# ChristianFeldmann/VTM

Hardware: AMD Instinct MI355X
Metric: hot-path pictures/sec (3840x2160 randomaccess QP32; level-order predInterSearch: AMVP estimation, TZ + fractional ME per (list, refIdx), bi refinement, MC, residual xT/quant/xIT/SSE; not a full encode) + SATD Gblocks/s (higher is better)
Workload: dtype int16 samples, int32 accumulation (fp64 MV-rate multiply)

## Files before the change

### include/vtmhip.h

```cpp
#ifndef VTMHIP_H
#define VTMHIP_H

#include <stddef.h>
#include <stdint.h>

#ifdef __cplusplus
extern "C" {
#endif

#define VTMHIP_ABI_VERSION 6

enum
{
  VTMHIP_OK            = 0,
  VTMHIP_E_INVALID     = -1,
  VTMHIP_E_NODEVICE    = -2,
  VTMHIP_E_HIP         = -3,
  VTMHIP_E_NOMEM       = -4,
  VTMHIP_E_UNSUPPORTED = -5
};

enum { VTMHIP_DIST_SAD = 0, VTMHIP_DIST_SATD = 1, VTMHIP_DIST_SSE = 2 };
enum { VTMHIP_DCT2 = 0, VTMHIP_DCT8 = 1, VTMHIP_DST7 = 2,
       VTMHIP_TRSKIP = 3 };
// ... 694 lines not shown

typedef struct
{
  const int16_t *org;
  const int16_t *dpb;
  int16_t *pred, *resi;
  int16_t *orgBi;
  int16_t *predC, *resiC;
} vtmhip_pis_buffers;

int vtmhip_pis_run_picture( vtmhip_ctx *ctx, const vtmhip_pis_level_run *levels, int numLevels, const vtmhip_pis_buffers *buf, void *mainStream,
                            void *const *sideStreams, int numSide );

int vtmhip_predInterSearch_batch_dev( vtmhip_ctx *ctx, const vtmhip_pis_level_run *L, const vtmhip_pis_buffers *buf );
int vtmhip_is_uniform_shape( int width, int height );

#ifdef __cplusplus
}
#endif
#endif
```

### vtm_amd/csrc/me.hip

```cpp
#include "ctx.hpp"
#include "mest_glue.hpp"
#include "mv_rules.hpp"

#include <cstdlib>

namespace
{

struct Range { int left, right, top, bottom; };

struct MeJob
{
  const int16_t *org;
  const int16_t *ref;
  int            orgStride, refStride, w, h, ss;
  unsigned       imvShift;
  int            predHor, predVer, costScale;
  double         lambda;
  int            horMin, horMax, verMin, verMax;
  int            seg, segsPerRow, items, lpc;
  int            lpcShift, sprShift;
  bool           narrow;
  bool           tiny;
  unsigned       bias;
// ... 222 lines not shown

struct TzState
{
  Range              sr;
  unsigned long long bestSad;
  int                bestX, bestY, pointNr;
  unsigned           bestDist, bestRound, nEval;
};

struct Coop
{
  int                 lane, wave, wpj;
  bool                leader;
  unsigned long long *redCost;
  unsigned           *redIdx;
};

template<int WPJ>
__device__ __forceinline__ void job_sync()
{
  if( WPJ == 1 )
  {
    __builtin_amdgcn_fence( __ATOMIC_ACQ_REL, "wavefront" );
    __builtin_amdgcn_wave_barrier();
  }
  else
  {
    __syncthreads();
  }
}
// ... 115 lines not shown
    if( lane == 0 ) { co.redCost[co.wave] = bestCost; co.redIdx[co.wave] = bestIdx; }
    __syncthreads();
#pragma unroll
    for( int w = 0; w < WPJ; w++ )
    {
      const unsigned long long oc = co.redCost[w];
      const unsigned           oi = co.redIdx[w];
      if( oc < bestCost || ( oc == bestCost && oi < bestIdx ) ) { bestCost = oc; bestIdx = oi; }
    }
    __syncthreads();
  }
  bestCost = uni( bestCost );
  bestIdx  = uni( bestIdx );
}

template<int WPJ>
__device__ __forceinline__ void tz_round( const MeJob &j, TzState &s, const int4 *pts, int n, const Coop &co, bool touchMeta )
{
  job_sync<WPJ>();
  unsigned long long cost;
  unsigned           idx;
  eval_candidates<false, WPJ>( j, pts, n, 0, 0, 1, 1, co, cost, idx );
  s.nEval += ( unsigned ) n;
  if( n > 0 && cost < s.bestSad )
  {
    const int4 p = pts[idx];
    s.bestSad    = cost;
    s.bestX      = uni( p.x );
    s.bestY      = uni( p.y );
    if( touchMeta )
    {
      s.bestDist  = ( unsigned ) uni( p.w );
      s.bestRound = 0;
      s.pointNr   = uni( p.z );
    }
  }
  job_sync<WPJ>();
}

#define PUSH( X, Y, NR, D ) do { if( co.leader ) pts[n] = make_int4( ( X ), ( Y ), ( NR ), ( D ) ); n++; } while( 0 )

__device__ int diamond_points( const Range &sr, int sx, int sy, int d, bool corners, int4 *pts, const Coop &co )
{
  int       n = 0;
  const int top = sy - d, bot = sy + d, left = sx - d, right = sx + d;
  if( d == 1 )
  {
    if( top >= sr.top )
    {
      if( corners && left >= sr.left ) PUSH( left, top, 1, d );
      PUSH( sx, top, 2, d );
      if( corners && right <= sr.right ) PUSH( right, top, 3, d );
// ... 53 lines not shown
      if( inside || yt >= sr.top )
      {
        if( inside || xl >= sr.left ) PUSH( xl, yt, 0, d );
        if( inside || xr <= sr.right ) PUSH( xr, yt, 0, d );
      }
      if( inside || yb <= sr.bottom )
      {
        if( inside || xl >= sr.left ) PUSH( xl, yb, 0, d );
        if( inside || xr <= sr.right ) PUSH( xr, yb, 0, d );
      }
    }
  }
  return n;
}

template<int WPJ>
__device__ __forceinline__ void tz_diamond( const MeJob &j, TzState &s, int sx, int sy, int d, bool corners, int4 *pts, const Coop &co )
{
  const int n = diamond_points( s.sr, sx, sy, d, corners, pts, co );
  s.bestRound += 1;
  tz_round<WPJ>( j, s, pts, n, co, true );
}

template<int WPJ>
__device__ __forceinline__ void tz_two_point( const MeJob &j, TzState &s, int4 *pts, const Coop &co )
{
  const int xo0[9] = { 0, -1, -1, 0, -1, +1, -1, -1, +1 }, xo1[9] = { 0, 0, +1, +1, -1, +1, 0, +1, 0 };
  const int yo0[9] = { 0, 0, -1, -1, +1, -1, 0, +1, 0 }, yo1[9] = { 0, -1, -1, 0, -1, +1, +1, +1, +1 };
  int       ax = 0, ay = 0, bx = 0, by = 0;
#pragma unroll
  for( int k = 0; k < 9; k++ )
    if( k == s.pointNr ) { ax = xo0[k]; ay = yo0[k]; bx = xo1[k]; by = yo1[k]; }
  const int x1 = s.bestX + ax, y1 = s.bestY + ay, x2 = s.bestX + bx, y2 = s.bestY + by;
  int       n  = 0;
  if( x1 >= s.sr.left && x1 <= s.sr.right && y1 >= s.sr.top && y1 <= s.sr.bottom ) PUSH( x1, y1, 0, 2 );
  if( x2 >= s.sr.left && x2 <= s.sr.right && y2 >= s.sr.top && y2 <= s.sr.bottom ) PUSH( x2, y2, 0, 2 );
  tz_round<WPJ>( j, s, pts, n, co, true );
}

template<int IPL, int WPJ>
__device__ __forceinline__ void raster_resident_org( const MeJob &j, int total, int rLeft, int rTop, int nx, int stepXY, const Coop &co,
                                                     unsigned long long &bestCost, unsigned &bestIdx )
{
  const int lane = co.lane;
  const long os = ( long ) j.orgStride << j.ss, cs = ( long ) j.refStride << j.ss;
  Pel8 o[IPL];
  int  off[IPL];
#pragma unroll
  for( int m = 0; m < IPL; m++ )
  {
    const int it = lane + 64 * m, r = it >> j.sprShift, x = ( it - ( r << j.sprShift ) ) << 3;
    o[m] = *reinterpret_cast<const Pel8 *>( j.org + r * os + x );
// ... 28 lines not shown
    if( lane == 0 ) { co.redCost[co.wave] = bestCost; co.redIdx[co.wave] = bestIdx; }
    __syncthreads();
#pragma unroll
    for( int w = 0; w < WPJ; w++ )
    {
      const unsigned long long oc = co.redCost[w];
      const unsigned           oi = co.redIdx[w];
      if( oc < bestCost || ( oc == bestCost && oi < bestIdx ) ) { bestCost = oc; bestIdx = oi; }
    }
    __syncthreads();
  }
  bestCost = uni( bestCost );
  bestIdx  = uni( bestIdx );
}

template<int WPJ>
__device__ __forceinline__ void tz_raster( const MeJob &j, TzState &s, const Range &r, int stepXY, const Coop &co )
{
  const int nx = r.right >= r.left ? ( r.right - r.left ) / stepXY + 1 : 0;
  const int ny = r.bottom >= r.top ? ( r.bottom - r.top ) / stepXY + 1 : 0;
  const int total = nx * ny;
  unsigned long long cost;
  unsigned           idx;
  const int  ipl  = j.items >> 6;
  const bool fits = total > 0 && j.lpc == 64 && j.seg == 8 && j.sprShift >= 0 && ( j.items & 63 ) == 0;
  if( false ) {}
  else if( WPJ >= 4 && fits && ipl == 4 ) raster_resident_org<4, WPJ>( j, total, r.left, r.top, nx, stepXY, co, cost, idx );
  else if( WPJ >= 2 && fits && ipl == 1 ) raster_resident_org<1, WPJ>( j, total, r.left, r.top, nx, stepXY, co, cost, idx );
  else eval_candidates<true, WPJ>( j, nullptr, total, r.left, r.top, nx > 0 ? nx : 1, stepXY, co, cost, idx );
  s.nEval += ( unsigned ) total;
  if( total > 0 && cost < s.bestSad )
  {
    const int ry = ( int ) idx / nx, rx = ( int ) idx - ry * nx;
    s.bestSad   = cost;
    s.bestX     = r.left + rx * stepXY;
    s.bestY     = r.top + ry * stepXY;
    s.bestDist  = ( unsigned ) stepXY;
    s.bestRound = 0;
    s.pointNr   = 0;
  }
}

struct TzSaved
// ... 197 lines not shown
      if( c < bc ) { bc = c; bi = ( unsigned ) i; }
    }
    wave_argmin( bc, bi );
    if( lane == 0 ) { sRedCost[wv] = bc; sRedIdx[wv] = bi; }
    __syncthreads();
    if( threadIdx.x == 0 )
    {
      for( int w = 1; w < 4; w++ )
        if( sRedCost[w] < bc || ( sRedCost[w] == bc && sRedIdx[w] < bi ) ) { bc = sRedCost[w]; bi = sRedIdx[w]; }
      sv.rasterCost = bc; sv.rasterIdx = bi;
    }
    __syncthreads();
  }
}

template<int WPJ>
__device__ __forceinline__ void tz_search_one( const vtmhip_pic_params &pic, const int16_t *__restrict__ orgBase, const int16_t *__restrict__ refBase,
                                               const vtmhip_tz_job *__restrict__ jobs, int numJobs, vtmhip_me_result *__restrict__ results, int mode, TzSaved *__restrict__ saved,
                                               int *__restrict__ list, int totCap, const MeFuse &fu, int blockIdxX, int gridDimX )
{
  constexpr int JOBS_PER_BLOCK = WPJ == 1 ? 4 : 1;
  __shared__ int4               sPts[JOBS_PER_BLOCK][16];
  __shared__ unsigned long long sRedCost[WPJ];
  __shared__ unsigned           sRedIdx[WPJ];
  __shared__ __attribute__( ( aligned( 16 ) ) ) int16_t sOrgLds[WPJ >= 4 ? ORG_LDS_CAP : WPJ == 2 ? ORG_LDS_CAP2 : 8];
  const int lane = threadIdx.x & 63, wv = uni( ( int ) ( threadIdx.x >> 6 ) );
  const int blk    = mode == 2 ? blockIdxX : xcd_order( blockIdxX, gridDimX );
  int       jobIdx = WPJ == 1 ? blk * 4 + wv : blk;
  if( mode == 2 )
  {
    if( jobIdx >= list[0] ) return;
    jobIdx = uni( list[1 + jobIdx] );
  }
  if( jobIdx >= numJobs ) return;
  __shared__ int sExtra[JOBS_PER_BLOCK][15][2];
  vtmhip_tz_job  tj;
  const int( *extra )[2];
// ... 43 lines not shown
    const vtmhip_tz_job *jp = jobs + jobIdx;
    if( uni( ( int ) jp->width ) == 0 ) return;
    tj.orgOff = jp->orgOff; tj.refOff = jp->refOff; tj.orgStride = jp->orgStride; tj.refStride = jp->refStride; tj.puX = jp->puX; tj.puY = jp->puY;
    tj.width = jp->width; tj.height = jp->height; tj.subShift = jp->subShift; tj.imvShift = jp->imvShift; tj.signedSamples = jp->signedSamples;
    tj.predHor = jp->predHor; tj.predVer = jp->predVer; tj.motionLambda = jp->motionLambda; tj.mvHor = jp->mvHor; tj.mvVer = jp->mvVer; tj.searchRange = jp->searchRange;
    tj.extendedSettings = jp->extendedSettings; tj.fastSettings = jp->fastSettings; tj.firstSearchStop = jp->firstSearchStop; tj.hasIntMv2Nx2NPred = jp->hasIntMv2Nx2NPred;
    tj.intMv2Nx2NPredHor = jp->intMv2Nx2NPredHor; tj.intMv2Nx2NPredVer = jp->intMv2Nx2NPredVer;
    numExtra = jp->numExtraStart;
    extra = jp->extraStart;
  }
  const vtmhip_tz_job *jp = &tj;
  int4                *pts = sPts[WPJ == 1 ? wv : 0];
  Coop                 co;
  co.lane = lane; co.wave = WPJ == 1 ? 0 : wv; co.wpj = WPJ; co.leader = ( lane == 0 && co.wave == 0 );
  co.redCost = sRedCost; co.redIdx = sRedIdx;

  MeJob j;
  j.org       = orgBase + jp->orgOff;
  j.ref       = refBase + jp->refOff;
  j.orgStride = jp->orgStride;
  j.refStride = jp->refStride;
  j.w         = jp->width;
  j.h         = jp->height;
  j.ss        = jp->subShift;
  j.imvShift  = ( unsigned ) jp->imvShift;
  j.predHor   = jp->predHor;
  j.predVer   = jp->predVer;
  j.costScale = 2;
  j.lambda    = jp->motionLambda;
  j.horMax    = MVR_CLIP_MAX( pic.picW, jp->puX );
// ... 20 lines not shown
    const int  r = j.sprShift >= 0 ? sub >> j.sprShift : sub / j.segsPerRow, x = ( sub - r * j.segsPerRow ) * j.seg;
    const long os = ( long ) j.orgStride << j.ss;
    if( j.seg == 8 )
    {
      const Pel8 a = *reinterpret_cast<const Pel8 *>( j.org + r * os + x );
#pragma unroll
      for( int k = 0; k < 4; k++ ) j.orgSeg[k] = a.v[k] ^ j.bias;
    }
    else
    {
      const Pel4 a = *reinterpret_cast<const Pel4 *>( j.org + r * os + x );
      j.orgSeg[0] = a.v[0] ^ j.bias; j.orgSeg[1] = a.v[1] ^ j.bias;
    }
    j.resOff = ( int ) ( r * ( ( long ) j.refStride << j.ss ) + x );
  }
  stage_org<WPJ, ( WPJ >= 4 ? ORG_LDS_CAP : ORG_LDS_CAP2 )>( j, sOrgLds, ( int ) threadIdx.x );

  const bool ext = jp->extendedSettings != 0, fast = jp->fastSettings != 0, firstStop = jp->firstSearchStop != 0;
  const int  iRaster = fast ? 8 : 5, searchRange = jp->searchRange;

  TzState s;
  s.bestSad = ~0ull; s.bestX = 0; s.bestY = 0; s.pointNr = 0; s.bestDist = 0; s.bestRound = 0; s.nEval = 0;
  s.sr.left = s.sr.right = s.sr.top = s.sr.bottom = 0;

  int startX = 0, startY = 0;
  if( mode != 2 )
  {
  int mx = jp->mvHor, my = jp->mvVer;
  clip_mv( j, mx, my );
  mx = div_pow2( mvr::prec_down( mx, 2 ), 2 );
  my = div_pow2( mvr::prec_down( my, 2 ), 2 );
  if( !jp->hasIntMv2Nx2NPred )
  {
    int n = 0;
    PUSH( mx, my, 0, 0 );
    if( !fast && ( mx != 0 || my != 0 ) ) PUSH( 0, 0, 0, 0 );
    const int ne = min( numExtra, 14 );
    for( int i = 0; i < ne; i++ )
    {
      int ex = extra[i][0], ey = extra[i][1];
      clip_mv( j, ex, ey );
      PUSH( mvr::prec_down( ex, 4 ), mvr::prec_down( ey, 4 ), 0, 0 );
    }
    tz_round<WPJ>( j, s, pts, n, co, true );
    if( numExtra > 14 )
    {
      int m = 0;
      {
        int n = 0;
        int ex = extra[14][0], ey = extra[14][1];
        clip_mv( j, ex, ey );
        PUSH( mvr::prec_down( ex, 4 ), mvr::prec_down( ey, 4 ), 0, 0 );
        m = n;
      }
      tz_round<WPJ>( j, s, pts, m, co, false );
    }
  }
  else
  {
    {
      int n = 0;
      PUSH( mx, my, 0, 0 );
      tz_round<WPJ>( j, s, pts, n, co, true );
    }
    if( !fast && ( mx != 0 || my != 0 ) && ( s.bestX != 0 || s.bestY != 0 ) )
    {
      int n = 0;
      PUSH( 0, 0, 0, 0 );
      tz_round<WPJ>( j, s, pts, n, co, true );
    }
    int ix = jp->intMv2Nx2NPredHor << 4, iy = jp->intMv2Nx2NPredVer << 4;
    clip_mv( j, ix, iy );
    ix = div_pow2( mvr::prec_down( ix, 2 ), 2 );
    iy = div_pow2( mvr::prec_down( iy, 2 ), 2 );
    if( ( mx != ix || my != iy ) && ( ix != s.bestX || iy != s.bestY ) )
    {
      int n = 0;
      PUSH( ix, iy, 0, 0 );
      tz_round<WPJ>( j, s, pts, n, co, true );
    }
    int       n  = 0;
    const int ne = min( numExtra, 15 );
    for( int i = 0; i < ne; i++ )
    {
      int ex = extra[i][0], ey = extra[i][1];
      clip_mv( j, ex, ey );
      PUSH( mvr::prec_down( ex, 4 ), mvr::prec_down( ey, 4 ), 0, 0 );
    }
    tz_round<WPJ>( j, s, pts, n, co, false );
  }

  s.sr = search_range( j, s.bestX << 4, s.bestY << 4, searchRange >> ( fast ? 1 : 0 ) );

  startX = s.bestX; startY = s.bestY;
  const bool bestCandidateZero = ( s.bestX == 0 && s.bestY == 0 );

  for( int d = 1; d <= searchRange; d *= 2 )
  {
    tz_diamond<WPJ>( j, s, startX, startY, d, ext, pts, co );
    if( firstStop && s.bestRound >= 3 ) break;
  }
  if( ext && !bestCandidateZero )
  {
    for( int d = 1; d <= ( searchRange >> 1 ); d *= 2 ) tz_diamond<WPJ>( j, s, 0, 0, d, false, pts, co );
  }
  if( s.bestDist == 1 )
  {
    s.bestDist = 0;
    tz_two_point<WPJ>( j, s, pts, co );
  }
  if( ext )
  {
    int   win = iRaster;
    Range lsr = s.sr;
    if( !( ( int ) s.bestDist >= iRaster ) )
    {
      win++;
      lsr.left /= 2; lsr.right /= 2; lsr.top /= 2; lsr.bottom /= 2;
    }
    s.bestDist = ( unsigned ) win;
    tz_raster<WPJ>( j, s, lsr, win, co );
  }
  else if( ( int ) s.bestDist >= iRaster )
  {
    s.bestDist = ( unsigned ) iRaster;
    const int nx = s.sr.right >= s.sr.left ? ( s.sr.right - s.sr.left ) / iRaster + 1 : 0, ny = s.sr.bottom >= s.sr.top ? ( s.sr.bottom - s.sr.top ) / iRaster + 1 : 0;
    if( mode == 1 && iRaster == 5 && j.seg == 8 && j.h <= 128 && nx >= 1 && ny >= 1 && nx * ny <= totCap )
    {
      if( co.leader )
      {
        TzSaved sv;
        sv.sr = s.sr; sv.bestSad = s.bestSad; sv.bestX = s.bestX; sv.bestY = s.bestY; sv.pointNr = s.pointNr; sv.bestDist = s.bestDist;
        sv.bestRound = s.bestRound; sv.nEval = s.nEval; sv.rasterCost = ~0ull; sv.rasterIdx = 0; sv.pad = 0;
        saved[jobIdx] = sv;
        list[1 + atomicAdd( &list[0], 1 )] = jobIdx;
      }
      if( fu.me && co.leader )
      {
        vtmhip_tz_job *g = fu.tzSpill + jobIdx;
        g->orgOff = tj.orgOff; g->refOff = tj.refOff; g->orgStride = tj.orgStride; g->refStride = tj.refStride; g->puX = tj.puX; g->puY = tj.puY;
        g->width = tj.width; g->height = tj.height; g->subShift = tj.subShift; g->imvShift = tj.imvShift; g->signedSamples = tj.signedSamples;
        g->predHor = tj.predHor; g->predVer = tj.predVer; g->motionLambda = tj.motionLambda; g->mvHor = tj.mvHor; g->mvVer = tj.mvVer; g->searchRange = tj.searchRange;
        g->extendedSettings = tj.extendedSettings; g->fastSettings = tj.fastSettings; g->firstSearchStop = tj.firstSearchStop; g->hasIntMv2Nx2NPred = tj.hasIntMv2Nx2NPred;
        g->intMv2Nx2NPredHor = tj.intMv2Nx2NPredHor; g->intMv2Nx2NPredVer = tj.intMv2Nx2NPredVer; g->numExtraStart = 0;
      }
      return;
    }
    tz_raster<WPJ>( j, s, s.sr, iRaster, co );
  }
  }
  else
  {
    const TzSaved sv = saved[jobIdx];
    s.sr = sv.sr; s.bestSad = uni( sv.bestSad ); s.bestX = uni( sv.bestX ); s.bestY = uni( sv.bestY ); s.pointNr = uni( sv.pointNr );
    s.bestDist = uni( sv.bestDist ); s.bestRound = uni( sv.bestRound ); s.nEval = uni( sv.nEval );
    s.sr.left = uni( s.sr.left ); s.sr.right = uni( s.sr.right ); s.sr.top = uni( s.sr.top ); s.sr.bottom = uni( s.sr.bottom );
    const int nx = ( s.sr.right - s.sr.left ) / 5 + 1, ny = ( s.sr.bottom - s.sr.top ) / 5 + 1;
    s.nEval += ( unsigned ) ( nx * ny );
    const unsigned long long rc = uni( sv.rasterCost );
    if( rc < s.bestSad )
    {
      const int idx = ( int ) uni( sv.rasterIdx ), ry = idx / nx, rx = idx - ry * nx;
      s.bestSad = rc; s.bestX = s.sr.left + rx * 5; s.bestY = s.sr.top + ry * 5; s.bestDist = 5; s.bestRound = 0; s.pointNr = 0;
    }
  }
  while( s.bestDist > 0 )
  {
    startX     = s.bestX;
    startY     = s.bestY;
    s.bestDist = 0;
    s.pointNr  = 0;
    for( int d = 1; d < searchRange + 1; d *= 2 )
    {
      tz_diamond<WPJ>( j, s, startX, startY, d, ext, pts, co );
      if( fast && s.bestRound >= 2 ) break;
    }
    if( s.bestDist == 1 )
    {
      s.bestDist = 0;
      if( s.pointNr != 0 ) tz_two_point<WPJ>( j, s, pts, co );
    }
  }

  if( co.leader )
  {
    vtmhip_me_result r;
    r.mvX = s.bestX; r.mvY = s.bestY; r.nEval = s.nEval; r.reserved = 0;
    r.cost = s.bestSad;
    r.dist = s.bestSad - mv_cost( j, s.bestX, s.bestY );
    results[jobIdx] = r;
  }
}

template<int WPJ>
__global__ __launch_bounds__( WPJ == 1 ? 256 : 64 * WPJ ) __attribute__( ( amdgpu_waves_per_eu( WPJ == 2 || WPJ == 4 || WPJ == 8 ? 4 : 1 ) ) )
void tz_search_kernel( vtmhip_pic_params pic, const int16_t *__restrict__ orgBase, const int16_t *__restrict__ refBase, const vtmhip_tz_job *__restrict__ jobs, int numJobs,
                       vtmhip_me_result *__restrict__ results, int mode, TzSaved *__restrict__ saved, int *__restrict__ list, int totCap, MeFuse fu )
{
  if( WPJ == 1 && mode == 2 )
  {
    const int listed = uni( list[0] );
    for( int b = ( int ) blockIdx.x; b * 4 < listed; b += ( int ) gridDim.x )
      tz_search_one<WPJ>( pic, orgBase, refBase, jobs, numJobs, results, mode, saved, list, totCap, fu, b, ( int ) gridDim.x );
    return;
  }
  tz_search_one<WPJ>( pic, orgBase, refBase, jobs, numJobs, results, mode, saved, list, totCap, fu, ( int ) blockIdx.x, ( int ) gridDim.x );
}


#ifndef VTMHIP_TZG_SPEC
#define VTMHIP_TZG_SPEC 1
#endif
#ifndef VTMHIP_TZG_WAVES
#define VTMHIP_TZG_WAVES 4
#endif
enum { GP_START = 0, GP_START15, GP_DIA1, GP_TWO1, GP_DIA2, GP_TWO2 };

template<int CTRL>
__device__ __forceinline__ unsigned long long dpp_u64( unsigned long long v )
{
  return ( ( unsigned long long ) dpp_u32<CTRL>( ( unsigned ) ( v >> 32 ) ) << 32 ) | dpp_u32<CTRL>( ( unsigned ) v );
// ... 614 lines not shown
    r.mvX = 0; r.mvY = 0; r.nEval = ( unsigned ) ( nx * ny ); r.reserved = 0; r.cost = ~0ull; r.dist = ~0ull;
    if( nx * ny > 0 )
    {
      const int idx = ( int ) sIdx[tid], ry = idx / nx, rx = idx - ry * nx;
      r.mvX  = sRange[tid][0] + rx;
      r.mvY  = sRange[tid][1] + ry;
      r.cost = sBest[tid];
      r.dist = r.cost - mv_cost( j, r.mvX, r.mvY );
    }
    results[job0 + tid] = r;
  }
}

}

extern "C" int vtmhip_tz_search_batch_dev( vtmhip_ctx *ctx, const vtmhip_pic_params *pic, const int16_t *d_orgBase, const int16_t *d_refBase,
                                           const vtmhip_tz_job *d_jobs, int n, vtmhip_me_result *d_results )
{
  return vtmhip_internal_tz_search( ctx, pic, d_orgBase, d_refBase, d_jobs, n, d_results, nullptr, 0, 0 );
}

int vtmhip_internal_tz_search( vtmhip_ctx *ctx, const vtmhip_pic_params *pic, const int16_t *d_orgBase, const int16_t *d_refBase, const vtmhip_tz_job *d_jobs, int n,
                               vtmhip_me_result *d_results, const MeFuse *fuse, int uniformW, int uniformH )
{
  VTMHIP_CHECK_CTX( ctx );
  VTMHIP_REQUIRE( ctx, pic && n >= 0, "pic / n" );
  if( n == 0 ) return VTMHIP_OK;
  VTMHIP_REQUIRE( ctx, d_orgBase && d_refBase && d_jobs && d_results, "null pointer" );
  MeFuse fuNone; memset( &fuNone, 0, sizeof( fuNone ) );
  const MeFuse fuFirst = fuse ? *fuse : fuNone;
// ... 15 lines not shown
    rasterParts = ( splitScan && n <= 640 ) ? ( 1280 / n < 8 ? 1280 / n : 8 ) : 1;
    if( totCap > RASTER_TOT_CAP && splitScan && n <= 4096 && rasterParts < 4 ) rasterParts = 4;
    const size_t oList = ( ( size_t ) n * sizeof( TzSaved ) + 255 ) & ~( size_t ) 255;
    const size_t oTot  = ( oList + ( ( size_t ) n + 1 ) * sizeof( int ) + 255 ) & ~( size_t ) 255;
    if( rasterParts > 1 && ( size_t ) n * ( totCap + 1 ) * sizeof( unsigned ) > ( ( size_t ) 64 << 20 ) ) rasterParts = 1;
    const size_t totBytes = rasterParts > 1 ? ( size_t ) n * ( totCap + 1 ) * sizeof( unsigned ) : 0;
    void        *arena = nullptr;
    int          st    = vtmhip_internal_workspace( ctx, oTot + totBytes, &arena, 1 );
    if( st ) return st;
    d_saved = ( TzSaved * ) arena;
    d_list  = ( int * ) ( ( char * ) arena + oList );
    d_tot   = ( unsigned * ) ( ( char * ) arena + oTot );
    if( totBytes ) VTMHIP_HIP( ctx, hipMemsetAsync( d_list, 0, ( size_t ) ( ( char * ) d_tot - ( char * ) d_list ) + totBytes, ctx->stream ) );
    else VTMHIP_HIP( ctx, hipMemsetAsync( d_list, 0, sizeof( int ), ctx->stream ) );
  }
#define VTMHIP_TZ_LAUNCH( W, GRID, MODE ) \
  hipLaunchKernelGGL( tz_search_kernel<W>, dim3( GRID ), dim3( W == 1 ? 256 : 64 * W ), 0, ctx->stream, *pic, d_orgBase, d_refBase, d_jobs, n, d_results, MODE, d_saved, d_list, totCap, \
                      ( MODE ) == 2 ? fuNone : fuFirst )
#define VTMHIP_TZ_SWITCH( MODE )                                    \
  switch( wpj )                                                     \
  {                                                                 \
  case 2: VTMHIP_TZ_LAUNCH( 2, n, MODE ); break;                    \
  case 4: VTMHIP_TZ_LAUNCH( 4, n, MODE ); break;                    \
  case 8: VTMHIP_TZ_LAUNCH( 8, n, MODE ); break;                    \
  case 16: VTMHIP_TZ_LAUNCH( 16, n, MODE ); break;                  \
  default: VTMHIP_TZ_LAUNCH( 1, ( ( MODE ) == 2 && ( n + 3 ) / 4 > 2048 ? 2048 : ( n + 3 ) / 4 ), MODE ); break; \
  }
  static const bool groupOn = !( getenv( "VTMHIP_TZ_GROUP" ) && atoi( getenv( "VTMHIP_TZ_GROUP" ) ) == 0 );
  static const int  groupItems = getenv( "VTMHIP_TZ_GROUP_ITEMS" ) ? atoi( getenv( "VTMHIP_TZ_GROUP_ITEMS" ) ) : 32;
  int grpItems = 0, grpSs = 0;
  if( groupOn && fuse && fuse->me && !fuse->cfg.extendedSettings && ( wpj == 0 || wpj == 1 ) && ( uniformW == 8 || uniformW == 16 || uniformW == 32 ) && uniformH >= 8 )
  {
    const int ss = fuse->cfg.fastInterSearchMode13 && uniformH > 8 && uniformW <= 64 ? 1 : 0;
    const int items = ( uniformW >> 3 ) * ( ( uniformH + ( 1 << ss ) - 1 ) >> ss );
    if( ( items & 7 ) == 0 && items <= groupItems && items <= 128 ) { grpItems = items; grpSs = ss; }
  }
  if( grpItems )
  {
    VTMHIP_TIME_KERNEL( ctx, "tz_group_kernel" );
    const int    spr = uniformW >> 3;
    const size_t lds = ( size_t ) 16 * grpItems * 16;
    const dim3   grid( ( n + 15 ) / 16 );
    const int    md = split ? 1 : 0;
#define VTMHIP_TZG_LAUNCH( SPR, SS )                                                                                                                                        \
  {                                                                                                                                                                         \
    if( lds > 48 * 1024 ) VTMHIP_HIP( ctx, hipFuncSetAttribute( reinterpret_cast<const void *>( tz_group_kernel<SPR, SS> ), hipFuncAttributeMaxDynamicSharedMemorySize, ( int ) lds ) ); \
    hipLaunchKernelGGL( ( tz_group_kernel<SPR, SS> ), grid, dim3( 256 ), lds, ctx->stream, *pic, d_orgBase, d_refBase, n, d_results, md, d_saved, d_list, totCap, grpItems, fuFirst ); \
  }
    if( spr == 1 && grpSs == 0 ) VTMHIP_TZG_LAUNCH( 1, 0 )
    else if( spr == 1 ) VTMHIP_TZG_LAUNCH( 1, 1 )
    else if( spr == 2 && grpSs == 0 ) VTMHIP_TZG_LAUNCH( 2, 0 )
    else if( spr == 2 ) VTMHIP_TZG_LAUNCH( 2, 1 )
    else if( grpSs == 0 ) VTMHIP_TZG_LAUNCH( 4, 0 )
    else VTMHIP_TZG_LAUNCH( 4, 1 )
#undef VTMHIP_TZG_LAUNCH
  }
  else
  { VTMHIP_TIME_KERNEL( ctx, "tz_search_kernel" );
    VTMHIP_TZ_SWITCH( split ? 1 : 0 )
  }
  if( split )
  {
    { VTMHIP_TIME_KERNEL( ctx, "tz_raster_cols_kernel" );
      const size_t totLds = ( size_t ) ( totCap + 1 ) * sizeof( unsigned );
      if( totLds > 32 * 1024 ) VTMHIP_HIP( ctx, hipFuncSetAttribute( reinterpret_cast<const void *>( tz_raster_cols_kernel ), hipFuncAttributeMaxDynamicSharedMemorySize, ( int ) totLds ) );
      hipLaunchKernelGGL( tz_raster_cols_kernel, dim3( rasterParts > 1 ? n * rasterParts : ( n < 3072 ? n : 3072 ) ), dim3( 256 ), totLds, ctx->stream, *pic, d_orgBase,
                          d_refBase, d_jobs, d_saved, d_list, d_tot, rasterParts, totCap );
    }
    { VTMHIP_TIME_KERNEL( ctx, "tz_search_kernel" );
      VTMHIP_TZ_SWITCH( 2 )
    }
  }
#undef VTMHIP_TZ_SWITCH
#undef VTMHIP_TZ_LAUNCH
  VTMHIP_LAUNCHED( ctx );
  return VTMHIP_OK;
}


static int full_search_uniform( vtmhip_ctx *ctx, const vtmhip_pic_params *pic, const int16_t *d_orgBase, const int16_t *d_refBase, const vtmhip_full_job *d_jobs, int n,
                                int width, int height, vtmhip_me_result *d_results, const FullFuse &fu );

extern "C" int vtmhip_full_search_batch_dev( vtmhip_ctx *ctx, const vtmhip_pic_params *pic, const int16_t *d_orgBase, const int16_t *d_refBase,
                                             const vtmhip_full_job *d_jobs, int n, vtmhip_me_result *d_results )
{
  return vtmhip_internal_full_search( ctx, pic, d_orgBase, d_refBase, d_jobs, n, 0, 0, d_results, nullptr );
}

int vtmhip_internal_full_search( vtmhip_ctx *ctx, const vtmhip_pic_params *pic, const int16_t *d_orgBase, const int16_t *d_refBase, const vtmhip_full_job *d_jobs, int n,
// ... 70 lines not shown
```

### vtm_amd/device.py

```python
import ctypes as C

import numpy as np

from . import lib as _lib
from .lib import (AffineJob, DistJob, FracJob, FracResult, FullJob, IfJob, McJob, MeResult, PelOpJob, PicParams, QuantJob,
                  TrJob, TuJob, TuResult, TzJob, VtmHipError, WpDistJob, WpParam, WpPredJob, WtdJob)


class DevBuf:

    def __init__(self, ctx, nbytes, dtype=np.uint8, shape=None):
        self.ctx = ctx
        self.nbytes = int(nbytes)
        self.dtype = np.dtype(dtype)
        self.shape = shape
        p = C.c_void_p()
        ctx._check(ctx.L.vtmhip_dev_alloc(ctx.h, self.nbytes, C.byref(p)))
        self.ptr = p.value
        ctx._bufs.append(self)

    def upload(self, arr):
        arr = np.ascontiguousarray(arr)
        assert arr.nbytes <= self.nbytes
        self.ctx._keep.append(arr)
# ... 216 lines not shown
                                                              max_w, max_h, d_results))

    def estimate_mvp_amvp_batch(self, pic, d_org, d_ref, d_jobs, n, max_w, max_h, uniform=False, add_idx_bits=True, d_dist_bip=None):
        self._check(self.L.vtmhip_xEstimateMvPredAMVP_batch_dev(self.h, C.byref(pic), d_org, d_ref, d_jobs, n, max_w, max_h, int(uniform), int(add_idx_bits), d_dist_bip))

    def pis_run_picture(self, levels, n_levels, buffers, main_stream, side_streams):
        arr = (C.c_void_p * max(1, len(side_streams)))(*side_streams)
        self._check(self.L.vtmhip_pis_run_picture(self.h, levels, n_levels, C.byref(buffers), C.c_void_p(main_stream), arr, len(side_streams)))

    def pred_inter_search_batch(self, level_run, buffers):
        self._check(self.L.vtmhip_predInterSearch_batch_dev(self.h, C.byref(level_run), C.byref(buffers)))

    def is_uniform_shape(self, w, h):
        return bool(self.L.vtmhip_is_uniform_shape(w, h))

    def affine_motion_estimation_batch(self, pic, d_org, d_ref, d_other, d_jobs, n, max_w, max_h, d_results, bcw=False):
        f = self.L.vtmhip_xAffineMotionEstimation_bcw_batch_dev if bcw else self.L.vtmhip_xAffineMotionEstimation_batch_dev
        self._check(f(self.h, C.byref(pic), d_org, d_ref, d_other, d_jobs, n, max_w, max_h, d_results))

    def mts_select_batch(self, d_results, num_tu, cands, w, h, bit_depth, max_cand, d_test):
        arr = (C.c_uint8 * 8)(*cands)
        self._check(self.L.vtmhip_mts_select_batch_dev(self.h, d_results, num_tu, len(cands), arr, w, h, bit_depth, 15, max_cand, d_test))

    def smvd_batch(self, pic, d_org, d_ref, d_jobs, n, max_w, max_h, op, uniform=False):
        fn = (self.L.vtmhip_xGetSymmetricCost_batch_dev, self.L.vtmhip_xSymmetricMotionEstimation_batch_dev, self.L.vtmhip_symmvdCheckBestMvp_batch_dev)
        if op < 3 and not uniform:
            self._check(fn[op](self.h, C.byref(pic), d_org, d_ref, d_jobs, n, max_w, max_h))
        else:
            self._check(self.L.vtmhip_smvd_batch_dev(self.h, C.byref(pic), d_org, d_ref, d_jobs, n, max_w, max_h, op | (0x100 if uniform else 0)))

# ... 88 lines not shown
```

### vtm_amd/lib.py

```python
import ctypes as C
import os

HERE = os.path.dirname(os.path.abspath(__file__))
LIB_PATH = os.path.join(HERE, "libvtmhip.so")

OK, E_INVALID, E_NODEVICE, E_HIP, E_NOMEM, E_UNSUPPORTED = 0, -1, -2, -3, -4, -5
DIST_SAD, DIST_SATD, DIST_SSE = 0, 1, 2
WTD_INV_RESHAPE_CUR = 1
WTD_INVALID_DIST = (1 << 64) - 1
WP_INVALID_DIST = (1 << 64) - 1
WP_UNI, WP_BI = 0, 1
DCT2, DCT8, DST7 = 0, 1, 2


class DistJob(C.Structure):
    _fields_ = [("orgOff", C.c_int64), ("curOff", C.c_int64), ("orgStride", C.c_int32), ("curStride", C.c_int32),
                ("width", C.c_int16), ("height", C.c_int16), ("subShift", C.c_int16), ("kind", C.c_int16)]


class PicParams(C.Structure):
    _fields_ = [("picW", C.c_int32), ("picH", C.c_int32), ("ctuSize", C.c_int32), ("bitDepth", C.c_int32),
                ("wavesPerJob", C.c_int32), ("maxSearchRange", C.c_int32)]


# ... 347 lines not shown
    "vtmhip_smvd_batch_dev": (C.c_int, [C.c_void_p, C.POINTER(PicParams), C.c_void_p, C.c_void_p, C.c_void_p, C.c_int, C.c_int, C.c_int, C.c_int]),
    "vtmhip_xGetSymmetricCost_batch_dev": (C.c_int, [C.c_void_p, C.POINTER(PicParams), C.c_void_p, C.c_void_p, C.c_void_p, C.c_int, C.c_int, C.c_int]),
    "vtmhip_xSymmetricMotionEstimation_batch_dev": (C.c_int, [C.c_void_p, C.POINTER(PicParams), C.c_void_p, C.c_void_p, C.c_void_p, C.c_int, C.c_int, C.c_int]),
    "vtmhip_symmvdCheckBestMvp_batch_dev": (C.c_int, [C.c_void_p, C.POINTER(PicParams), C.c_void_p, C.c_void_p, C.c_void_p, C.c_int, C.c_int, C.c_int]),
    "vtmhip_xPredAffineBlk_batch_dev": (C.c_int, [C.c_void_p, C.POINTER(PicParams), C.c_void_p, C.c_void_p, C.c_void_p, C.c_int, C.c_int, C.c_int]),
    "vtmhip_lfnst_tu_batch_dev": (C.c_int, [C.c_void_p, C.c_void_p, C.c_void_p, C.c_int]),
    "vtmhip_lfnst_scan_host": (C.c_int, [C.c_int, C.c_int, C.c_void_p]),
    "vtmhip_kernel_timing": (C.c_int, [C.c_void_p, C.c_int]),
    "vtmhip_kernel_timing_read": (C.c_int, [C.c_void_p, C.c_char_p, C.POINTER(C.c_double), C.POINTER(C.c_int)]),
    "vtmhip_merge_cand_satd_batch_dev": (C.c_int, [C.c_void_p, C.POINTER(PicParams), C.c_void_p, C.c_void_p, C.c_void_p, C.c_void_p, C.c_int, C.c_void_p, C.c_int,
                                                   C.c_void_p, C.c_int, C.c_void_p, C.c_int, C.c_int, C.c_int, C.c_int, C.c_void_p]),
    "vtmhip_pis_run_picture": (C.c_int, [C.c_void_p, C.POINTER(PisLevelRun), C.c_int, C.POINTER(PisBuffers), C.c_void_p, C.POINTER(C.c_void_p), C.c_int]),
    "vtmhip_pis_stage": (C.c_int, [C.c_void_p, C.POINTER(PisLevel), C.c_int]),
    "vtmhip_predInterSearch_batch_dev": (C.c_int, [C.c_void_p, C.POINTER(PisLevelRun), C.POINTER(PisBuffers)]),
    "vtmhip_is_uniform_shape": (C.c_int, [C.c_int, C.c_int]),
    "vtmhip_tz_search_batch_dev": (C.c_int, [C.c_void_p, C.POINTER(PicParams), C.c_void_p, C.c_void_p, C.c_void_p,
                                             C.c_int, C.c_void_p]),
}

_lib = None


class VtmHipError(RuntimeError):
    def __init__(self, status, detail=""):
        self.status = status
        super().__init__("libvtmhip status %d%s" % (status, (": " + detail) if detail else ""))


def _share_hip_runtime_with_torch():
    try:
# ... 35 lines not shown
```

Measured before the change: 88.32.

## Add register-resident org band path for TZ candidate rounds

Adds a templated band mode (K items per thread) where the original block is held in registers and each round's candidates are evaluated by all lanes via readlane-broadcast positions. Per-candidate SADs are reduced with DPP and written to double-buffered LDS partials, so one barrier per round replaces two. Rasters also get an LDS-staged org path. It is selected at launch for uniform shapes that tile exactly, and it costs more template instantiations, register pressure and code size.

```diff
diff --git a/include/vtmhip.h b/include/vtmhip.h
--- a/include/vtmhip.h
+++ b/include/vtmhip.h
@@ -732,6 +732,7 @@
 
 int vtmhip_predInterSearch_batch_dev( vtmhip_ctx *ctx, const vtmhip_pis_level_run *L, const vtmhip_pis_buffers *buf );
 int vtmhip_is_uniform_shape( int width, int height );
+int vtmhip_tz_band_items( int width, int height, int subShift, int wavesPerJob );
 
 #ifdef __cplusplus
 }
diff --git a/vtm_amd/csrc/me.hip b/vtm_amd/csrc/me.hip
--- a/vtm_amd/csrc/me.hip
+++ b/vtm_amd/csrc/me.hip
@@ -260,6 +260,9 @@
   bool                leader;
   unsigned long long *redCost;
   unsigned           *redIdx;
+  int4               *ptsBase;
+  unsigned           *part;
+  int16_t            *orgLds;
 };
 
 template<int WPJ>
@@ -405,13 +408,145 @@
   bestIdx  = uni( bestIdx );
 }
 
-template<int WPJ>
-__device__ __forceinline__ void tz_round( const MeJob &j, TzState &s, const int4 *pts, int n, const Coop &co, bool touchMeta )
-{
+constexpr int BAND_LOADS = 8;
+
+template<int K> struct Band
+{
+  unsigned o[K > 0 ? K : 1][4];
+  unsigned offB, stepB;
+};
+
+template<int K>
+__device__ __forceinline__ void band_load_org( const MeJob &j, Band<K> &bd, int tid, int threads )
+{
+  const int  r = tid >> j.sprShift, x = ( tid & ( j.segsPerRow - 1 ) ) << 3;
+  const long os = ( long ) j.orgStride << j.ss;
+  const int  cs = j.refStride << j.ss, rows = threads >> j.sprShift;
+#pragma unroll
+  for( int m = 0; m < K; m++ )
+  {
+    const Pel8 a = *reinterpret_cast<const Pel8 *>( j.org + ( r + m * rows ) * os + x );
+#pragma unroll
+    for( int k = 0; k < 4; k++ ) bd.o[m][k] = a.v[k] ^ j.bias;
+  }
+  bd.offB  = ( unsigned ) ( r * cs + x ) * 2u;
+  bd.stepB = ( unsigned ) ( rows * cs ) * 2u;
+}
+
+template<int K, bool SGN>
+__device__ __forceinline__ unsigned band_partials( const MeJob &j, const Band<K> &bd, int px, int py, int n, int lane )
+{
+  constexpr int  CH = K == 4 ? 1 : BAND_LOADS / K;
+  const bool   evenStride = !( ( j.refStride << j.ss ) & 1 );
+  const size_t stepB = uni( bd.stepB );
+  const int    slot = lane & 15;
+  unsigned     mine = 0;
+  for( int c0 = 0; c0 < n; c0 += CH )
+  {
+    Pel8     b[CH][K];
+    unsigned e[CH][K];
+    bool     odd[CH];
+#pragma unroll
+    for( int q = 0; q < CH; q++ )
+    {
+      odd[q] = false;
+      if( c0 + q < n )
+      {
+        const int16_t *cp = j.ref + ( long ) __builtin_amdgcn_readlane( py, c0 + q ) * j.refStride + __builtin_amdgcn_readlane( px, c0 + q );
+        odd[q] = evenStride && ( reinterpret_cast<uintptr_t>( cp ) & 2 ) != 0;
+        const char *cb = reinterpret_cast<const char *>( cp ) - ( odd[q] ? 2 : 0 );
+#pragma unroll
+        for( int m = 0; m < K; m++ ) b[q][m] = *reinterpret_cast<const Pel8 *>( cb + m * stepB + bd.offB );
+        if( odd[q] )
+        {
+#pragma unroll
+          for( int m = 0; m < K; m++ ) e[q][m] = *reinterpret_cast<const unsigned *>( cb + m * stepB + 16 + bd.offB );
+        }
+      }
+    }
+#pragma unroll
+    for( int q = 0; q < CH; q++ )
+      if( c0 + q < n )
+      {
+        if( odd[q] )
+        {
+#pragma unroll
+          for( int m = 0; m < K; m++ )
+          {
+            Pel8 &v = b[q][m];
+            v.v[0] = __builtin_amdgcn_alignbit( v.v[1], v.v[0], 16 ); v.v[1] = __builtin_amdgcn_alignbit( v.v[2], v.v[1], 16 );
+            v.v[2] = __builtin_amdgcn_alignbit( v.v[3], v.v[2], 16 ); v.v[3] = __builtin_amdgcn_alignbit( e[q][m], v.v[3], 16 );
+          }
+        }
+        unsigned s = 0;
+#pragma unroll
+        for( int m = 0; m < K; m++ )
+#pragma unroll
+          for( int k = 0; k < 4; k++ ) s = sad2( bd.o[m][k], bx<SGN>( b[q][m].v[k], j.bias ), s );
+        s += dpp_u32<DPP_XOR1>( s );
+        s += dpp_u32<DPP_XOR2>( s );
+        s += dpp_u32<DPP_HALF_MIRROR>( s );
+        s += dpp_u32<DPP_MIRROR>( s );
+        mine = slot == c0 + q ? s : mine;
+      }
+  }
+  return mine;
+}
+
+template<int WPJ, int K>
+__device__ __forceinline__ void band_round( const MeJob &j, const Band<K> &bd, const int4 *pts, int n, const Coop &co, unsigned long long &bestCost, unsigned &bestIdx )
+{
+  const int lane = co.lane;
+  unsigned *part = co.part + ( pts == co.ptsBase ? 0 : 16 * 4 * WPJ );
+  const int4     p    = pts[lane & 15];
+  const unsigned mine = j.bias ? band_partials<K, true>( j, bd, p.x, p.y, n, lane ) : band_partials<K, false>( j, bd, p.x, p.y, n, lane );
+  if( ( lane & 15 ) < n ) part[( lane & 15 ) * ( 4 * WPJ ) + co.wave * 4 + ( lane >> 4 )] = mine;
+  job_sync<WPJ>();
+  constexpr int G = WPJ >= 4 ? 4 : 1;
+  unsigned      tot = 0;
+  {
+    const uint4 *pp = reinterpret_cast<const uint4 *>( part + ( G == 4 ? lane & 15 : min( lane, 15 ) ) * ( 4 * WPJ ) ) + ( G == 4 ? ( lane >> 4 ) * ( WPJ / 4 ) : 0 );
+#pragma unroll
+    for( int w = 0; w < WPJ / G; w++ ) { const uint4 t = pp[w]; tot += t.x + t.y + t.z + t.w; }
+    if( G == 4 ) { tot += __shfl_xor( tot, 16, 64 ); tot += __shfl_xor( tot, 32, 64 ); }
+  }
+  const bool valid = lane < n;
+  bestCost = ~0ull;
+  bestIdx  = valid ? ( unsigned ) lane : 0xffffffffu;
+  if( valid ) bestCost = ( ( unsigned long long ) tot << j.ss ) + mv_cost( j, p.x, p.y );
+  if( j.narrow )
+  {
+    unsigned cm, km;
+    if( j.tiny )
+    {
+      const unsigned m = wave_min_u32( valid ? ( ( unsigned ) bestCost << 6 ) | bestIdx : 0xffffffffu );
+      cm = m == 0xffffffffu ? 0xffffffffu : m >> 6;
+      km = m == 0xffffffffu ? 0xffffffffu : m & 63u;
+    }
+    else
+    {
+      const unsigned c32 = valid ? ( unsigned ) bestCost : 0xffffffffu;
+      cm = wave_min_u32( c32 );
+      km = wave_min_u32( c32 == cm ? bestIdx : 0xffffffffu );
+    }
+    bestCost = km == 0xffffffffu ? ~0ull : ( unsigned long long ) uni( cm );
+    bestIdx  = uni( km );
+    return;
+  }
+  wave_argmin( bestCost, bestIdx );
+  bestCost = uni( bestCost );
+  bestIdx  = uni( bestIdx );
+}
+
+template<int WPJ, int K>
+__device__ __forceinline__ void tz_round( const MeJob &j, const Band<K> &bd, TzState &s, int4 *&pts, int n, const Coop &co, bool touchMeta )
+{
+  if( K > 0 && n == 0 ) return;
   job_sync<WPJ>();
   unsigned long long cost;
   unsigned           idx;
-  eval_candidates<false, WPJ>( j, pts, n, 0, 0, 1, 1, co, cost, idx );
+  if constexpr( K > 0 ) band_round<WPJ, K>( j, bd, pts, n, co, cost, idx );
+  else eval_candidates<false, WPJ>( j, pts, n, 0, 0, 1, 1, co, cost, idx );
   s.nEval += ( unsigned ) n;
   if( n > 0 && cost < s.bestSad )
   {
@@ -426,7 +561,8 @@
       s.pointNr   = uni( p.z );
     }
   }
-  job_sync<WPJ>();
+  if constexpr( K > 0 ) pts = co.ptsBase + ( pts == co.ptsBase ? 16 : 0 );
+  else job_sync<WPJ>();
 }
 
 #define PUSH( X, Y, NR, D ) do { if( co.leader ) pts[n] = make_int4( ( X ), ( Y ), ( NR ), ( D ) ); n++; } while( 0 )
@@ -510,16 +646,16 @@
   return n;
 }
 
-template<int WPJ>
-__device__ __forceinline__ void tz_diamond( const MeJob &j, TzState &s, int sx, int sy, int d, bool corners, int4 *pts, const Coop &co )
+template<int WPJ, int K>
+__device__ __forceinline__ void tz_diamond( const MeJob &j, const Band<K> &bd, TzState &s, int sx, int sy, int d, bool corners, int4 *&pts, const Coop &co )
 {
   const int n = diamond_points( s.sr, sx, sy, d, corners, pts, co );
   s.bestRound += 1;
-  tz_round<WPJ>( j, s, pts, n, co, true );
-}
-
-template<int WPJ>
-__device__ __forceinline__ void tz_two_point( const MeJob &j, TzState &s, int4 *pts, const Coop &co )
+  tz_round<WPJ, K>( j, bd, s, pts, n, co, true );
+}
+
+template<int WPJ, int K>
+__device__ __forceinline__ void tz_two_point( const MeJob &j, const Band<K> &bd, TzState &s, int4 *&pts, const Coop &co )
 {
   const int xo0[9] = { 0, -1, -1, 0, -1, +1, -1, -1, +1 }, xo1[9] = { 0, 0, +1, +1, -1, +1, 0, +1, 0 };
   const int yo0[9] = { 0, 0, -1, -1, +1, -1, 0, +1, 0 }, yo1[9] = { 0, -1, -1, 0, -1, +1, +1, +1, +1 };
@@ -531,7 +667,7 @@
   int       n  = 0;
   if( x1 >= s.sr.left && x1 <= s.sr.right && y1 >= s.sr.top && y1 <= s.sr.bottom ) PUSH( x1, y1, 0, 2 );
   if( x2 >= s.sr.left && x2 <= s.sr.right && y2 >= s.sr.top && y2 <= s.sr.bottom ) PUSH( x2, y2, 0, 2 );
-  tz_round<WPJ>( j, s, pts, n, co, true );
+  tz_round<WPJ, K>( j, bd, s, pts, n, co, true );
 }
 
 template<int IPL, int WPJ>
@@ -590,7 +726,7 @@
   bestIdx  = uni( bestIdx );
 }
 
-template<int WPJ>
+template<int WPJ, int K>
 __device__ __forceinline__ void tz_raster( const MeJob &j, TzState &s, const Range &r, int stepXY, const Coop &co )
 {
   const int nx = r.right >= r.left ? ( r.right - r.left ) / stepXY + 1 : 0;
@@ -603,6 +739,12 @@
   if( false ) {}
   else if( WPJ >= 4 && fits && ipl == 4 ) raster_resident_org<4, WPJ>( j, total, r.left, r.top, nx, stepXY, co, cost, idx );
   else if( WPJ >= 2 && fits && ipl == 1 ) raster_resident_org<1, WPJ>( j, total, r.left, r.top, nx, stepXY, co, cost, idx );
+  else if( K > 0 && WPJ >= 2 && total > 0 )
+  {
+    MeJob js = j;
+    stage_org<WPJ, ( WPJ >= 4 ? ORG_LDS_CAP : ORG_LDS_CAP2 )>( js, co.orgLds, co.lane + 64 * co.wave );
+    eval_candidates<true, WPJ>( js, nullptr, total, r.left, r.top, nx, stepXY, co, cost, idx );
+  }
   else eval_candidates<true, WPJ>( j, nullptr, total, r.left, r.top, nx > 0 ? nx : 1, stepXY, co, cost, idx );
   s.nEval += ( unsigned ) total;
   if( total > 0 && cost < s.bestSad )
@@ -830,13 +972,14 @@
   }
 }
 
-template<int WPJ>
+template<int WPJ, int K>
 __device__ __forceinline__ void tz_search_one( const vtmhip_pic_params &pic, const int16_t *__restrict__ orgBase, const int16_t *__restrict__ refBase,
                                                const vtmhip_tz_job *__restrict__ jobs, int numJobs, vtmhip_me_result *__restrict__ results, int mode, TzSaved *__restrict__ saved,
                                                int *__restrict__ list, int totCap, const MeFuse &fu, int blockIdxX, int gridDimX )
 {
   constexpr int JOBS_PER_BLOCK = WPJ == 1 ? 4 : 1;
-  __shared__ int4               sPts[JOBS_PER_BLOCK][16];
+  __shared__ int4               sPts[JOBS_PER_BLOCK][K > 0 ? 32 : 16];
+  __shared__ __attribute__( ( aligned( 16 ) ) ) unsigned sPart[K > 0 ? JOBS_PER_BLOCK * 2 * 16 * 4 * WPJ : 1];
   __shared__ unsigned long long sRedCost[WPJ];
   __shared__ unsigned           sRedIdx[WPJ];
   __shared__ __attribute__( ( aligned( 16 ) ) ) int16_t sOrgLds[WPJ >= 4 ? ORG_LDS_CAP : WPJ == 2 ? ORG_LDS_CAP2 : 8];
@@ -910,6 +1053,7 @@
   Coop                 co;
   co.lane = lane; co.wave = WPJ == 1 ? 0 : wv; co.wpj = WPJ; co.leader = ( lane == 0 && co.wave == 0 );
   co.redCost = sRedCost; co.redIdx = sRedIdx;
+  co.ptsBase = pts; co.part = sPart + ( WPJ == 1 ? wv : 0 ) * ( 2 * 16 * 4 * WPJ ); co.orgLds = sOrgLds;
 
   MeJob j;
   j.org       = orgBase + jp->orgOff;
@@ -960,7 +1104,15 @@
     }
     j.resOff = ( int ) ( r * ( ( long ) j.refStride << j.ss ) + x );
   }
-  stage_org<WPJ, ( WPJ >= 4 ? ORG_LDS_CAP : ORG_LDS_CAP2 )>( j, sOrgLds, ( int ) threadIdx.x );
+  Band<K> bd;
+  if constexpr( K > 0 )
+  {
+    if( j.seg != 8 || j.sprShift < 0 || j.items != K * 64 * WPJ ) return;
+    j.orgLds = nullptr;
+    if( K == 1 && WPJ == 1 ) { bd.o[0][0] = j.orgSeg[0]; bd.o[0][1] = j.orgSeg[1]; bd.o[0][2] = j.orgSeg[2]; bd.o[0][3] = j.orgSeg[3]; bd.offB = ( unsigned ) j.resOff * 2u; bd.stepB = 0; }
+    else band_load_org<K>( j, bd, WPJ == 1 ? lane : ( int ) threadIdx.x, 64 * WPJ );
+  }
+  else stage_org<WPJ, ( WPJ >= 4 ? ORG_LDS_CAP : ORG_LDS_CAP2 )>( j, sOrgLds, ( int ) threadIdx.x );
 
   const bool ext = jp->extendedSettings != 0, fast = jp->fastSettings != 0, firstStop = jp->firstSearchStop != 0;
   const int  iRaster = fast ? 8 : 5, searchRange = jp->searchRange;
@@ -988,7 +1140,7 @@
       clip_mv( j, ex, ey );
       PUSH( mvr::prec_down( ex, 4 ), mvr::prec_down( ey, 4 ), 0, 0 );
     }
-    tz_round<WPJ>( j, s, pts, n, co, true );
+    tz_round<WPJ, K>( j, bd, s, pts, n, co, true );
     if( numExtra > 14 )
     {
       int m = 0;
@@ -999,7 +1151,7 @@
         PUSH( mvr::prec_down( ex, 4 ), mvr::prec_down( ey, 4 ), 0, 0 );
         m = n;
       }
-      tz_round<WPJ>( j, s, pts, m, co, false );
+      tz_round<WPJ, K>( j, bd, s, pts, m, co, false );
     }
   }
   else
@@ -1007,13 +1159,13 @@
     {
       int n = 0;
       PUSH( mx, my, 0, 0 );
-      tz_round<WPJ>( j, s, pts, n, co, true );
+      tz_round<WPJ, K>( j, bd, s, pts, n, co, true );
     }
     if( !fast && ( mx != 0 || my != 0 ) && ( s.bestX != 0 || s.bestY != 0 ) )
     {
       int n = 0;
       PUSH( 0, 0, 0, 0 );
-      tz_round<WPJ>( j, s, pts, n, co, true );
+      tz_round<WPJ, K>( j, bd, s, pts, n, co, true );
     }
     int ix = jp->intMv2Nx2NPredHor << 4, iy = jp->intMv2Nx2NPredVer << 4;
     clip_mv( j, ix, iy );
@@ -1023,7 +1175,7 @@
     {
       int n = 0;
       PUSH( ix, iy, 0, 0 );
-      tz_round<WPJ>( j, s, pts, n, co, true );
+      tz_round<WPJ, K>( j, bd, s, pts, n, co, true );
     }
     int       n  = 0;
     const int ne = min( numExtra, 15 );
@@ -1033,7 +1185,7 @@
       clip_mv( j, ex, ey );
       PUSH( mvr::prec_down( ex, 4 ), mvr::prec_down( ey, 4 ), 0, 0 );
     }
-    tz_round<WPJ>( j, s, pts, n, co, false );
+    tz_round<WPJ, K>( j, bd, s, pts, n, co, false );
   }
 
   s.sr = search_range( j, s.bestX << 4, s.bestY << 4, searchRange >> ( fast ? 1 : 0 ) );
@@ -1043,17 +1195,17 @@
 
   for( int d = 1; d <= searchRange; d *= 2 )
   {
-    tz_diamond<WPJ>( j, s, startX, startY, d, ext, pts, co );
+    tz_diamond<WPJ, K>( j, bd, s, startX, startY, d, ext, pts, co );
     if( firstStop && s.bestRound >= 3 ) break;
   }
   if( ext && !bestCandidateZero )
   {
-    for( int d = 1; d <= ( searchRange >> 1 ); d *= 2 ) tz_diamond<WPJ>( j, s, 0, 0, d, false, pts, co );
+    for( int d = 1; d <= ( searchRange >> 1 ); d *= 2 ) tz_diamond<WPJ, K>( j, bd, s, 0, 0, d, false, pts, co );
   }
   if( s.bestDist == 1 )
   {
     s.bestDist = 0;
-    tz_two_point<WPJ>( j, s, pts, co );
+    tz_two_point<WPJ, K>( j, bd, s, pts, co );
   }
   if( ext )
   {
@@ -1065,7 +1217,7 @@
       lsr.left /= 2; lsr.right /= 2; lsr.top /= 2; lsr.bottom /= 2;
     }
     s.bestDist = ( unsigned ) win;
-    tz_raster<WPJ>( j, s, lsr, win, co );
+    tz_raster<WPJ, K>( j, s, lsr, win, co );
   }
   else if( ( int ) s.bestDist >= iRaster )
   {
@@ -1092,7 +1244,7 @@
       }
       return;
     }
-    tz_raster<WPJ>( j, s, s.sr, iRaster, co );
+    tz_raster<WPJ, K>( j, s, s.sr, iRaster, co );
   }
   }
   else
@@ -1118,13 +1270,13 @@
     s.pointNr  = 0;
     for( int d = 1; d < searchRange + 1; d *= 2 )
     {
-      tz_diamond<WPJ>( j, s, startX, startY, d, ext, pts, co );
+      tz_diamond<WPJ, K>( j, bd, s, startX, startY, d, ext, pts, co );
       if( fast && s.bestRound >= 2 ) break;
     }
     if( s.bestDist == 1 )
     {
       s.bestDist = 0;
-      if( s.pointNr != 0 ) tz_two_point<WPJ>( j, s, pts, co );
+      if( s.pointNr != 0 ) tz_two_point<WPJ, K>( j, bd, s, pts, co );
     }
   }
 
@@ -1138,8 +1290,8 @@
   }
 }
 
-template<int WPJ>
-__global__ __launch_bounds__( WPJ == 1 ? 256 : 64 * WPJ ) __attribute__( ( amdgpu_waves_per_eu( WPJ == 2 || WPJ == 4 || WPJ == 8 ? 4 : 1 ) ) )
+template<int WPJ, int K = 0>
+__global__ __launch_bounds__( WPJ == 1 ? 256 : 64 * WPJ ) __attribute__( ( amdgpu_waves_per_eu( WPJ == 2 || WPJ == 4 || WPJ == 8 || ( K > 0 && WPJ > 1 ) ? 4 : 1 ) ) )
 void tz_search_kernel( vtmhip_pic_params pic, const int16_t *__restrict__ orgBase, const int16_t *__restrict__ refBase, const vtmhip_tz_job *__restrict__ jobs, int numJobs,
                        vtmhip_me_result *__restrict__ results, int mode, TzSaved *__restrict__ saved, int *__restrict__ list, int totCap, MeFuse fu )
 {
@@ -1147,10 +1299,10 @@
   {
     const int listed = uni( list[0] );
     for( int b = ( int ) blockIdx.x; b * 4 < listed; b += ( int ) gridDim.x )
-      tz_search_one<WPJ>( pic, orgBase, refBase, jobs, numJobs, results, mode, saved, list, totCap, fu, b, ( int ) gridDim.x );
+      tz_search_one<WPJ, K>( pic, orgBase, refBase, jobs, numJobs, results, mode, saved, list, totCap, fu, b, ( int ) gridDim.x );
     return;
   }
-  tz_search_one<WPJ>( pic, orgBase, refBase, jobs, numJobs, results, mode, saved, list, totCap, fu, ( int ) blockIdx.x, ( int ) gridDim.x );
+  tz_search_one<WPJ, K>( pic, orgBase, refBase, jobs, numJobs, results, mode, saved, list, totCap, fu, ( int ) blockIdx.x, ( int ) gridDim.x );
 }
 
 
@@ -1795,6 +1947,21 @@
 
 }
 
+extern "C" int vtmhip_tz_band_items( int width, int height, int subShift, int wavesPerJob )
+{
+  const int wpj = wavesPerJob <= 1 ? 1 : wavesPerJob;
+  if( wpj != 1 && wpj != 2 && wpj != 4 && wpj != 8 && wpj != 16 ) return 0;
+  if( width < 8 || ( width & 7 ) || height < 1 || subShift < 0 || subShift > 1 ) return 0;
+  const int spr = width >> 3, threads = 64 * wpj;
+  if( ( spr & ( spr - 1 ) ) || spr > 64 ) return 0;
+  const int items = spr * ( ( height + ( 1 << subShift ) - 1 ) >> subShift );
+  if( items % threads ) return 0;
+  const int k = items / threads;
+  if( wpj == 1 && k != 1 ) return 0;
+  if( wpj == 16 && k == 4 ) return 0;
+  return k == 1 || k == 2 || k == 4 ? k : 0;
+}
+
 extern "C" int vtmhip_tz_search_batch_dev( vtmhip_ctx *ctx, const vtmhip_pic_params *pic, const int16_t *d_orgBase, const int16_t *d_refBase,
                                            const vtmhip_tz_job *d_jobs, int n, vtmhip_me_result *d_results )
 {
@@ -1840,9 +2007,17 @@
     if( totBytes ) VTMHIP_HIP( ctx, hipMemsetAsync( d_list, 0, ( size_t ) ( ( char * ) d_tot - ( char * ) d_list ) + totBytes, ctx->stream ) );
     else VTMHIP_HIP( ctx, hipMemsetAsync( d_list, 0, sizeof( int ), ctx->stream ) );
   }
-#define VTMHIP_TZ_LAUNCH( W, GRID, MODE ) \
-  hipLaunchKernelGGL( tz_search_kernel<W>, dim3( GRID ), dim3( W == 1 ? 256 : 64 * W ), 0, ctx->stream, *pic, d_orgBase, d_refBase, d_jobs, n, d_results, MODE, d_saved, d_list, totCap, \
+#define VTMHIP_TZ_LAUNCH_K( W, KK, GRID, MODE ) \
+  hipLaunchKernelGGL( ( tz_search_kernel<W, KK> ), dim3( GRID ), dim3( W == 1 ? 256 : 64 * W ), 0, ctx->stream, *pic, d_orgBase, d_refBase, d_jobs, n, d_results, MODE, d_saved, d_list, totCap, \
                       ( MODE ) == 2 ? fuNone : fuFirst )
+#define VTMHIP_TZ_LAUNCH( W, GRID, MODE )                               \
+  switch( bandK )                                                       \
+  {                                                                     \
+  case 1: VTMHIP_TZ_LAUNCH_K( W, 1, GRID, MODE ); break;                \
+  case 2: VTMHIP_TZ_LAUNCH_K( W, ( W == 1 ? 0 : 2 ), GRID, MODE ); break; \
+  case 4: VTMHIP_TZ_LAUNCH_K( W, ( W == 1 || W == 16 ? 0 : 4 ), GRID, MODE ); break; \
+  default: VTMHIP_TZ_LAUNCH_K( W, 0, GRID, MODE ); break;               \
+  }
 #define VTMHIP_TZ_SWITCH( MODE )                                    \
   switch( wpj )                                                     \
   {                                                                 \
@@ -1855,6 +2030,8 @@
   static const bool groupOn = !( getenv( "VTMHIP_TZ_GROUP" ) && atoi( getenv( "VTMHIP_TZ_GROUP" ) ) == 0 );
   static const int  groupItems = getenv( "VTMHIP_TZ_GROUP_ITEMS" ) ? atoi( getenv( "VTMHIP_TZ_GROUP_ITEMS" ) ) : 32;
   int grpItems = 0, grpSs = 0;
+  static const bool bandsOn = !( getenv( "VTMHIP_TZ_BANDS" ) && atoi( getenv( "VTMHIP_TZ_BANDS" ) ) == 0 );
+  int bandK = 0;
   if( groupOn && fuse && fuse->me && !fuse->cfg.extendedSettings && ( wpj == 0 || wpj == 1 ) && ( uniformW == 8 || uniformW == 16 || uniformW == 32 ) && uniformH >= 8 )
   {
     const int ss = fuse->cfg.fastInterSearchMode13 && uniformH > 8 && uniformW <= 64 ? 1 : 0;
@@ -1883,6 +2060,8 @@
   }
   else
   { VTMHIP_TIME_KERNEL( ctx, "tz_search_kernel" );
+    if( bandsOn && fuse && fuse->me && uniformW > 0 && uniformH > 0 )
+      bandK = vtmhip_tz_band_items( uniformW, uniformH, fuse->cfg.fastInterSearchMode13 && uniformH > 8 && uniformW <= 64 ? 1 : 0 , wpj );
     VTMHIP_TZ_SWITCH( split ? 1 : 0 )
   }
   if( split )
@@ -1899,6 +2078,7 @@
   }
 #undef VTMHIP_TZ_SWITCH
 #undef VTMHIP_TZ_LAUNCH
+#undef VTMHIP_TZ_LAUNCH_K
   VTMHIP_LAUNCHED( ctx );
   return VTMHIP_OK;
 }
diff --git a/vtm_amd/device.py b/vtm_amd/device.py
--- a/vtm_amd/device.py
+++ b/vtm_amd/device.py
@@ -254,6 +254,9 @@
     def is_uniform_shape(self, w, h):
         return bool(self.L.vtmhip_is_uniform_shape(w, h))
 
+    def tz_band_items(self, w, h, sub_shift, waves_per_job):
+        return int(self.L.vtmhip_tz_band_items(w, h, sub_shift, waves_per_job))
+
     def affine_motion_estimation_batch(self, pic, d_org, d_ref, d_other, d_jobs, n, max_w, max_h, d_results, bcw=False):
         f = self.L.vtmhip_xAffineMotionEstimation_bcw_batch_dev if bcw else self.L.vtmhip_xAffineMotionEstimation_batch_dev
         self._check(f(self.h, C.byref(pic), d_org, d_ref, d_other, d_jobs, n, max_w, max_h, d_results))
diff --git a/vtm_amd/lib.py b/vtm_amd/lib.py
--- a/vtm_amd/lib.py
+++ b/vtm_amd/lib.py
@@ -385,6 +385,7 @@
     "vtmhip_pis_stage": (C.c_int, [C.c_void_p, C.POINTER(PisLevel), C.c_int]),
     "vtmhip_predInterSearch_batch_dev": (C.c_int, [C.c_void_p, C.POINTER(PisLevelRun), C.POINTER(PisBuffers)]),
     "vtmhip_is_uniform_shape": (C.c_int, [C.c_int, C.c_int]),
+    "vtmhip_tz_band_items": (C.c_int, [C.c_int, C.c_int, C.c_int, C.c_int]),
     "vtmhip_tz_search_batch_dev": (C.c_int, [C.c_void_p, C.POINTER(PicParams), C.c_void_p, C.c_void_p, C.c_void_p,
                                              C.c_int, C.c_void_p]),
 }
```

After: 89.47 (median of 6 runs). 1.01x the previous value.
